# annappo/GPS-SDR-Receiver

Measured on AMD Instinct MI355X. Metric: IQ Msamples/s ingested, 32-SV acq + 12-ch track, higher is better.
Workload: dtype f32

## Files before the change

### gps-sdr-receiver_amd/csrc/gpsmi_fft.h

```cpp
#pragma once
#include <hip/hip_runtime.h>

namespace gpsmi {

__device__ __forceinline__ void lds_barrier() {
    asm volatile("s_waitcnt lgkmcnt(0)\n\ts_barrier" ::: "memory");
}


constexpr int kFftN = 2048;
constexpr int kFftThreads = 256;
constexpr int kFftPlane = kFftN + kFftN / 32;
constexpr int kFftPlane1 = kFftN + 8 * (kFftN / 64);
constexpr int kFftLdsFloats = 2 * kFftPlane + 2 * kFftPlane1;

__device__ __forceinline__ int fft_pad(int i) { return i + (i >> 5); }
__device__ __forceinline__ int fft_pad1(int i) { return i + 8 * (i >> 6); }

typedef float fft_c __attribute__((ext_vector_type(2)));

__device__ __forceinline__ fft_c cadd_mi(fft_c a, fft_c b) {
    fft_c d;
    asm("v_pk_add_f32 %0, %1, %2 op_sel:[0,1] op_sel_hi:[1,0] neg_hi:[0,1]" : "=v"(d) : "v"(a), "v"(b));
    return d;
}
__device__ __forceinline__ fft_c cadd_pi(fft_c a, fft_c b) {
    fft_c d;
    asm("v_pk_add_f32 %0, %1, %2 op_sel:[0,1] op_sel_hi:[1,0] neg_lo:[0,1]" : "=v"(d) : "v"(a), "v"(b));
    return d;
}
__device__ __forceinline__ fft_c cneg_add_mi(fft_c a) {
    fft_c d;
    asm("v_pk_add_f32 %0, %1, %1 op_sel:[0,1] op_sel_hi:[1,0] neg_lo:[1,0] neg_hi:[1,1]" : "=v"(d) : "v"(a));
    return d;
}
__device__ __forceinline__ fft_c cmulp(fft_c a, fft_c w) {
    fft_c d;
    asm("v_pk_mul_f32 %0, %2, %1 op_sel_hi:[1,0]\n\t"
        "v_pk_fma_f32 %0, %2, %1, %0 op_sel:[1,1,0] op_sel_hi:[0,1,1] neg_lo:[1,0,0]"
        : "=&v"(d) : "v"(a), "v"(w));
    return d;
}

__device__ __forceinline__ fft_c cmulp_conj(fft_c a, fft_c w) {
    fft_c d;
    asm("v_pk_mul_f32 %0, %2, %1 op_sel_hi:[1,0]\n\t"
        "v_pk_fma_f32 %0, %2, %1, %0 op_sel:[1,1,0] op_sel_hi:[0,1,1] neg_hi:[1,0,0]"
        : "=&v"(d) : "v"(a), "v"(w));
    return d;
}

template <bool B2MI>
__device__ __forceinline__ void dft4p(fft_c& b0, fft_c& b1, fft_c& b2, fft_c& b3) {
    const fft_c c0 = B2MI ? cadd_mi(b0, b2) : b0 + b2;
    const fft_c c1 = B2MI ? cadd_pi(b0, b2) : b0 - b2;
    const fft_c c2 = b1 + b3, d = b1 - b3;
    b0 = c0 + c2;
    b2 = c0 - c2;
    b1 = cadd_mi(c1, d);
    b3 = cadd_pi(c1, d);
}

__device__ __forceinline__ void dft8p(fft_c* v) {
    const float h = 0.70710678118654752440f;
    fft_c a0 = v[0] + v[4], a4 = v[0] - v[4];
    fft_c a1 = v[1] + v[5], a5 = v[1] - v[5];
    fft_c a2 = v[2] + v[6], a6 = v[2] - v[6];
    fft_c a3 = v[3] + v[7], a7 = v[3] - v[7];
    a5 = cadd_mi(a5, a5) * h;
    a7 = cneg_add_mi(a7) * h;
    dft4p<false>(a0, a1, a2, a3);
    dft4p<true>(a4, a5, a6, a7);
    v[0] = a0; v[2] = a1; v[4] = a2; v[6] = a3;
    v[1] = a4; v[3] = a5; v[5] = a6; v[7] = a7;
}

constexpr int kFftTwFloats = 2 * (64 + 512);
struct FftTw {
    const fft_c* t64;
    const fft_c* t512;
    fft_c w4[2][3];
};

__device__ __forceinline__ FftTw fft_setup(float* lds_tw, const float2* __restrict__ tw, int t) {
    float2* t64 = reinterpret_cast<float2*>(lds_tw);
    float2* t512 = t64 + 64;
    t64[t & 63] = tw[32 * (t & 63)];
    t512[t] = tw[4 * t];
    t512[t + 256] = tw[4 * (t + 256)];
    FftTw f;
    f.t64 = reinterpret_cast<const fft_c*>(t64);
    f.t512 = reinterpret_cast<const fft_c*>(t512);
#pragma unroll
    for (int b = 0; b < 2; ++b)
#pragma unroll
        for (int r = 1; r <= 3; ++r) {
            const float2 w = tw[r * (t + 256 * b)];
            f.w4[b][r - 1] = fft_c{w.x, w.y};
        }
    return f;
}

__device__ __forceinline__ void fft2048(float2* vio, float* lds, const FftTw& tw, int t) {
    fft_c* buf0 = reinterpret_cast<fft_c*>(lds);
    fft_c* buf1 = buf0 + kFftPlane;
    fft_c v[8];
#pragma unroll
    for (int r = 0; r < 8; ++r) v[r] = fft_c{vio[r].x, vio[r].y};

    dft8p(v);
#pragma unroll
    for (int r = 0; r < 8; ++r) buf0[fft_pad(8 * t + r)] = v[r];
    lds_barrier();
#pragma unroll
    for (int r = 0; r < 8; ++r) v[r] = buf0[fft_pad(t + 256 * r)];
    {
        const int k = t & 7;
#pragma unroll
        for (int r = 1; r < 8; ++r) v[r] = cmulp(v[r], tw.t64[r * k]);
        dft8p(v);
        const int base = (t >> 3) * 64 + k;
#pragma unroll
        for (int r = 0; r < 8; ++r) buf1[fft_pad1(base + 8 * r)] = v[r];
    }
    lds_barrier();
#pragma unroll
    for (int r = 0; r < 8; ++r) v[r] = buf1[fft_pad1(t + 256 * r)];
    {
        const int k = t & 63;
#pragma unroll
        for (int r = 1; r < 8; ++r) v[r] = cmulp(v[r], tw.t512[r * k]);
        dft8p(v);
        const int base = (t >> 6) * 512 + k;
#pragma unroll
        for (int r = 0; r < 8; ++r) buf0[fft_pad(base + 64 * r)] = v[r];
    }
    lds_barrier();
#pragma unroll
    for (int r = 0; r < 8; ++r) v[r] = buf0[fft_pad(t + 256 * r)];
#pragma unroll
    for (int b = 0; b < 2; ++b) {
        fft_c z1 = cmulp(v[b + 2], tw.w4[b][0]);
        fft_c z2 = cmulp(v[b + 4], tw.w4[b][1]);
        fft_c z3 = cmulp(v[b + 6], tw.w4[b][2]);
        fft_c z0 = v[b];
        dft4p<false>(z0, z1, z2, z3);
        v[b] = z0; v[b + 2] = z1; v[b + 4] = z2; v[b + 6] = z3;
    }
#pragma unroll
    for (int r = 0; r < 8; ++r) vio[r] = make_float2(v[r].x, v[r].y);
}

}
```

### gps-sdr-receiver_amd/csrc/gpsmi_stats.h

```cpp
#pragma once
#include <hip/hip_runtime.h>

#include "gpsmi_fft.h"

namespace gpsmi {

template <int CTRL, int ROWS>
__device__ __forceinline__ float dpp_add0(float v) {
    const float o = __builtin_bit_cast(
        float, __builtin_amdgcn_update_dpp(0, __builtin_bit_cast(int, v), CTRL, ROWS, 0xF, false));
    return v + o;
}
__device__ __forceinline__ float wave_sum_dpp(float v) {
    v = dpp_add0<0xB1, 0xF>(v);
    v = dpp_add0<0x4E, 0xF>(v);
    v = dpp_add0<0x141, 0xF>(v);
    v = dpp_add0<0x140, 0xF>(v);
    v = dpp_add0<0x142, 0xA>(v);
    v = dpp_add0<0x143, 0xC>(v);
    return __builtin_bit_cast(float, __builtin_amdgcn_readlane(__builtin_bit_cast(int, v), 63));
}

template <int CTRL>
__device__ __forceinline__ double dpp_add_f64(double v) {
    const long long b = __builtin_bit_cast(long long, v);
    const int lo = __builtin_amdgcn_update_dpp(0, (int)(b & 0xffffffffll), CTRL, 0xF, 0xF, false);
    const int hi = __builtin_amdgcn_update_dpp(0, (int)(b >> 32), CTRL, 0xF, 0xF, false);
    return v + __builtin_bit_cast(double, ((long long)hi << 32) | (unsigned)lo);
}
__device__ __forceinline__ double row_sum_f64_dpp(double v) {
    v = dpp_add_f64<0xB1>(v);
    v = dpp_add_f64<0x4E>(v);
    v = dpp_add_f64<0x141>(v);
    v = dpp_add_f64<0x140>(v);
    return v;
}

template <int CTRL, int ROWS>
__device__ __forceinline__ float dpp_max_own(float v) {
    const int vi = __builtin_bit_cast(int, v);
    return fmaxf(v, __builtin_bit_cast(float, __builtin_amdgcn_update_dpp(vi, vi, CTRL, ROWS, 0xF, false)));
}
template <int CTRL, int ROWS>
__device__ __forceinline__ int dpp_min_own(int v) {
    return min(v, __builtin_amdgcn_update_dpp(v, v, CTRL, ROWS, 0xF, false));
}
__device__ __forceinline__ void wave_argmax_dpp(float& v, int& i) {
    float m = v;
    m = dpp_max_own<0xB1, 0xF>(m);
    m = dpp_max_own<0x4E, 0xF>(m);
    m = dpp_max_own<0x141, 0xF>(m);
    m = dpp_max_own<0x140, 0xF>(m);
    m = dpp_max_own<0x142, 0xA>(m);
    m = dpp_max_own<0x143, 0xC>(m);
    m = __builtin_bit_cast(float, __builtin_amdgcn_readlane(__builtin_bit_cast(int, m), 63));
    int k = v == m ? i : 0x7fffffff;
    k = dpp_min_own<0xB1, 0xF>(k);
    k = dpp_min_own<0x4E, 0xF>(k);
    k = dpp_min_own<0x141, 0xF>(k);
    k = dpp_min_own<0x140, 0xF>(k);
    k = dpp_min_own<0x142, 0xA>(k);
    k = dpp_min_own<0x143, 0xC>(k);
    v = m;
    i = __builtin_amdgcn_readlane(k, 63);
}

constexpr int kStatsRedFloats = 16;

__device__ __forceinline__ void corr_stats8(const float* mag, int t, float* magbuf, float* red,
                                            int& amax, float& peak, float& mean, float& sd,
                                            float& lo, float& hi) {
    constexpr int N = 2048;
    const int wave = t >> 6, lane = t & 63;
    float sm = 0.f, bv = mag[0];
    int bi = t;
#pragma unroll
    for (int q = 0; q < 8; ++q) {
        sm += mag[q];
        if (mag[q] > bv) { bv = mag[q]; bi = t + 256 * q; }
        magbuf[t + 256 * q] = mag[q];
    }
    sm = wave_sum_dpp(sm);
    wave_argmax_dpp(bv, bi);
    if (lane == 0) { red[wave] = sm; red[4 + wave] = bv; ((int*)red)[8 + wave] = bi; }
    lds_barrier();
    sm = (red[0] + red[1]) + (red[2] + red[3]);
    bv = red[4]; bi = ((int*)red)[8];
#pragma unroll
    for (int w = 1; w < 4; ++w) {
        const float ov = red[4 + w];
        const int oi = ((int*)red)[8 + w];
        if (ov > bv || (ov == bv && oi < bi)) { bv = ov; bi = oi; }
    }
    mean = sm * (1.0f / N);
    float d2 = 0.f;
#pragma unroll
    for (int q = 0; q < 8; ++q) { const float d = mag[q] - mean; d2 += d * d; }
    d2 = wave_sum_dpp(d2);
    if (lane == 0) red[12 + wave] = d2;
    lds_barrier();
    d2 = (red[12] + red[13]) + (red[14] + red[15]);
    sd = sqrtf(d2 * (1.0f / N));
    amax = bi;
    peak = bv;
    lo = magbuf[(bi + N - 1) & (N - 1)];
    hi = magbuf[(bi + 1) & (N - 1)];
}

}
```

### gps-sdr-receiver_amd/csrc/gpsmi_trk.hip

```cpp
#include <atomic>
#include <chrono>
#include <cmath>
#include <condition_variable>
#include <cstdlib>
#include <cstring>
#include <deque>
#include <mutex>
#include <thread>
#include <vector>

#include <hip/hip_ext.h>

#include "gpsmi_common.h"
#include "gpsmi_fft.h"

#pragma clang fp contract(off)

namespace gpsmi {

constexpr float kTwoPiF = 6.28318530717958647692f;
constexpr float kPiF = 3.14159265358979323846f;

struct TrkParams {
    int cs;
// ... 663 lines not shown
    float2* d_rep = nullptr;
    float* d_code = nullptr;
    bool have_rep[GPSMI_MAX_PRN + 1] = {};
    float2* d_block = nullptr;
    gpsmi_trk_state* d_state = nullptr;
    std::vector<gpsmi_trk_state> h_state;
    bool state_dirty_host = false;
    size_t njobs_cap = 0;
    gpsmi_trk_state* d_tab_in = nullptr;
    gpsmi_trk_state* d_tab_out = nullptr;
    int* d_forced = nullptr;
    float last_total_ms = 0.f, last_corr_ms = 0.f, last_cp_ms = 0.f;
    int replay_nb = 0;
    bool replay_forced = false;
    int corr_cg = 4;
    int corr_small1 = 384, corr_small2 = 1536;
    int done_by_dispatch = 1;
    bool general = false;
    static constexpr int stream_j = 8;
    int mfma = 0;
    int codephase = 0;
    int corr_overlap = 0;
    int fold_chunk = 0;
    int epilogue_form = 1;
    float* d_code_eo = nullptr;
    int n_cu = 256;
    int iq_fmt = GPSMI_IQ_C64;
    int nchunks = 1;
    float2* d_fold = nullptr; float* d_mag = nullptr; DirStats* d_stats = nullptr;
    int* d_xsel = nullptr; int* d_rsel = nullptr; float2* d_partial_g = nullptr;
    bool big = false;
    float2* d_twN = nullptr; float2* d_RS = nullptr; float2* d_S = nullptr;
    bool pfa = false;
    float2* d_RSp = nullptr;
    bool span8 = false;
    TrkParams P;
    struct StreamJob { const void* iq; size_t n; gpsmi_trk_out* out; };
    struct StreamWorker {
        std::thread th;
        std::mutex m;
        std::condition_variable cv_job, cv_done;
        std::deque<StreamJob> q;
        bool stop = false;
        long long submitted = 0;
        long long cleared = 0;
        long long finished = 0;
        std::atomic<long long> a_submitted{0}, a_cleared{0}, a_finished{0};
        int err = 0;
        char errmsg[512] = "";
    };
    StreamWorker* worker = nullptr;
    int stream_thread = 1;
    int stream_depth = 2;
    long long stat_backlog = 0;
    long long stat_quiesce_ns = 0, stat_evwait_ns = 0, stat_waits = 0;
    long long stat_wait_ns = 0, stat_launch_ns = 0, stat_steps = 0;
};

constexpr int kSpanUnitsMax = 256;

static int trk_reserve(gpsmi_trk* h, size_t njobs) {
    if (njobs <= h->njobs_cap) return GPSMI_OK;
    void* olds[] = {h->d_tab_in, h->d_tab_out, h->d_forced, h->slot[0].d_mid, h->slot[1].d_mid,
                    h->slot[0].d_partial, h->slot[1].d_partial, h->slot[0].d_out, h->slot[1].d_out,
                    h->d_fold, h->d_mag, h->d_stats, h->d_xsel, h->d_rsel, h->d_partial_g,
                    h->slot[0].d_rec, h->slot[1].d_rec};
    for (void* p : olds)
        if (p) GPSMI_HIP(hipFree(p));
    h->d_tab_in = h->d_tab_out = nullptr; h->d_forced = nullptr;
    for (auto& sl : h->slot) { sl.d_mid = nullptr; sl.d_partial = nullptr; sl.d_out = nullptr; sl.d_rec = nullptr; }
    h->njobs_cap = 0;
    h->d_fold = nullptr; h->d_mag = nullptr; h->d_stats = nullptr; h->d_xsel = h->d_rsel = nullptr;
    h->d_partial_g = nullptr;
    if (h->mfma == 4)
        for (auto& sl : h->slot)
            GPSMI_HIP(hipMalloc((void**)&sl.d_rec, (size_t)kSpanUnitsMax * 32 * kSpRecFloats * sizeof(float)));
    if (h->general) {
        const size_t cs = h->cfg.code_samples;
        GPSMI_HIP(hipMalloc((void**)&h->d_fold, njobs * cs * sizeof(float2)));
        if (!h->pfa) GPSMI_HIP(hipMalloc((void**)&h->d_mag, njobs * cs * sizeof(float)));
        GPSMI_HIP(hipMalloc((void**)&h->d_stats, njobs * sizeof(DirStats)));
        GPSMI_HIP(hipMalloc((void**)&h->d_xsel, njobs * sizeof(int)));
        GPSMI_HIP(hipMalloc((void**)&h->d_rsel, njobs * sizeof(int)));
    }
    if (h->span8) {
        const size_t units = ((njobs + h->max_ch - 1) / h->max_ch) * ((h->max_ch + kSpCh - 1) / kSpCh);
        for (auto& sl : h->slot)
            GPSMI_HIP(hipMalloc((void**)&sl.d_rec, units * kS8Ranges * kS8RecFloats * sizeof(float)));
    }
    if (h->nchunks > 1 && !h->span8)
        GPSMI_HIP(hipMalloc((void**)&h->d_partial_g,
                            njobs * h->nchunks * (h->cfg.n_cyc + 1) * sizeof(float2)));
    GPSMI_HIP(hipMalloc((void**)&h->d_tab_in, njobs * sizeof(gpsmi_trk_state)));
    GPSMI_HIP(hipMalloc((void**)&h->d_tab_out, njobs * sizeof(gpsmi_trk_state)));
    GPSMI_HIP(hipMalloc((void**)&h->d_forced, njobs * sizeof(int)));
    for (auto& sl : h->slot) {
        GPSMI_HIP(hipMalloc((void**)&sl.d_mid, njobs * sizeof(JobMid)));
        GPSMI_HIP(hipMalloc((void**)&sl.d_partial, njobs * (h->cfg.n_cyc + 1) * sizeof(float2)));
        GPSMI_HIP(hipMalloc((void**)&sl.d_out, njobs * sizeof(gpsmi_trk_out)));
    }
    h->njobs_cap = njobs;
    return GPSMI_OK;
}

static int trk_launch(gpsmi_trk* h, gpsmi_trk::Slot& sl, const void* d_iq_v,
                      const gpsmi_trk_state* st_in, gpsmi_trk_state* st_out, const int* forced,
                      int njobs, int nch, bool side_epilogue = false, hipEvent_t tail_stop = nullptr,
                      bool* tail_stop_used = nullptr) {
    TrkParams P = h->P;
    P.nch = nch;
    hipStream_t rs = sl.run_stream ? sl.run_stream : h->stream;
    h->main_tail = nullptr;
    const float2* d_iq = static_cast<const float2*>(d_iq_v);
    const bool u8 = h->iq_fmt == GPSMI_IQ_U8;
    sl.corr_stop = sl.ev[2];
    const bool timed = h->timing == 1;
    const bool corr_stamps = h->timing == 2;
    if (timed) GPSMI_HIP(hipEventRecord(sl.ev[0], rs));
    const int nblocks = njobs / nch;
    const int ngroups = (nch + kGroupCh - 1) / kGroupCh;
    const dim3 sgrid(((nblocks + 7) / 8) * 8 * ngroups);
    const int ng_span = (nch + kSpCh - 1) / kSpCh;
    const bool span_single = h->mfma == 4 && nblocks * ng_span <= h->span_single_max;
    if (h->general) {
        const int cs = P.cs;
        const int chunk = (h->pfa && h->fold_chunk > 0 && h->fold_chunk < nblocks) ? h->fold_chunk : nblocks;
        for (int b0 = 0; b0 < nblocks; b0 += chunk) {
            const int nbc = nblocks - b0 < chunk ? nblocks - b0 : chunk;
            hipLaunchKernelGGL(trk_fold_general_kernel, dim3((cs + 255) / 256, nbc), dim3(256), 0,
                               rs, d_iq, h->d_t32, st_in, P, h->d_fold, h->d_xsel, h->d_rsel,
                               sl.d_mid, b0);
            if (h->pfa)
                pfa_corr_launch(rs, h->d_fold, h->d_xsel, h->d_rsel, nbc * nch, h->d_RSp, h->d_stats, b0 * nch);
        }
        if (h->pfa) {
        } else if (h->big)
            big_corr_launch(rs, h->d_fold, h->d_xsel, h->d_rsel, njobs, cs, h->d_RS, h->d_S,
                            h->d_tw, h->d_twN, h->d_mag);
        else
            hipLaunchKernelGGL(circ_corr_direct_kernel,
                               dim3((cs + kDirLagsPerWg - 1) / kDirLagsPerWg, njobs), dim3(256), 0,
                               rs, h->d_fold, h->d_code, h->d_xsel, h->d_rsel, cs,
                               h->d_mag);
        if (!h->pfa)
            hipLaunchKernelGGL(corr_stats_kernel, dim3(njobs), dim3(256), 0, rs, h->d_mag, cs,
                               h->d_stats);
        hipLaunchKernelGGL(trk_decide_kernel, dim3((njobs + 255) / 256), dim3(256), 0, rs,
                           h->d_stats, forced, P, njobs, sl.d_out, sl.d_mid);
    } else {
        const int jobs_all = nblocks * nch;
        const int cg = jobs_all <= h->corr_small1 ? 1 : (jobs_all <= h->corr_small2 ? 2 : h->corr_cg);
        const int ng = (nch + cg - 1) / cg;
        const dim3 cgrid(corr_grid(nblocks, ng));
#define GPSMI_LAUNCH_CORR(CGV)                                                                          \
    do {                                                                                              \
        if (u8)                                                                                       \
            hipLaunchKernelGGL((trk_corr_kernel<CGV, 1>), cgrid, dim3(256), 0, rs, d_iq_v,     \
                               st_in, forced, h->d_rep, h->d_tw, P, ng, nblocks, sl.d_out, sl.d_mid); \
        else                                                                                          \
            hipLaunchKernelGGL((trk_corr_kernel<CGV, 0>), cgrid, dim3(256), 0, rs, d_iq_v,     \
                               st_in, forced, h->d_rep, h->d_tw, P, ng, nblocks, sl.d_out, sl.d_mid); \
    } while (0)
        if (cg == 6) GPSMI_LAUNCH_CORR(6);
        else if (cg == 4) GPSMI_LAUNCH_CORR(4);
        else if (cg == 2) GPSMI_LAUNCH_CORR(2);
        else GPSMI_LAUNCH_CORR(1);
#undef GPSMI_LAUNCH_CORR
    }
    const bool ext_timed = (timed || corr_stamps) && h->mfma == 4 && !span_single;
    bool corr_done_recorded = false;
    const int span_units = nblocks * ng_span, span_slots = sp_wg_per_cu(P.n_cyc) * h->n_cu;
    const int span_per = (span_units + span_slots - 1) / span_slots;
    const dim3 span_grid((span_units + span_per - 1) / (span_per > 0 ? span_per : 1));
    if (timed && !ext_timed) GPSMI_HIP(hipEventRecord(sl.ev[1], rs));
    if (h->mfma) {
        const int ng12 = (nch + kSpCh - 1) / kSpCh;
        const JobMid* cmid = sl.d_mid;
        const float* ceo = h->d_code_eo;
#define GPSMI_LAUNCH_SPAN(NSP, WV, FMTV, NCV, GRID, BLOCK)                                                     \
    do {                                                                                                      \
        if (ext_timed && (NSP) == 8)                                                                          \
            hipExtLaunchKernelGGL((trk_span_kernel<NSP, WV, FMTV, 0, NCV>), GRID, BLOCK, 0, rs, sl.ev[1],     \
                                  sl.corr_stop, 0, d_iq_v, cmid, ceo, P, ng12, nblocks, sl.d_rec,             \
                                  sl.d_partial);                                                              \
        else if (by_dispatch && (NSP) == 8)                                                                   \
            hipExtLaunchKernelGGL((trk_span_kernel<NSP, WV, FMTV, 0, NCV>), GRID, BLOCK, 0, rs, nullptr,      \
                                  sl.corr_done, 0, d_iq_v, cmid, ceo, P, ng12, nblocks, sl.d_rec,             \
                                  sl.d_partial);                                                              \
        else                                                                                                  \
            hipLaunchKernelGGL((trk_span_kernel<NSP, WV, FMTV, 0, NCV>), GRID, BLOCK, 0, rs, d_iq_v, cmid,    \
                               ceo, P, ng12, nblocks, sl.d_rec, sl.d_partial);                                \
    } while (0)
#define GPSMI_LAUNCH_SPAN_NC(NCV)                                                                       \
    do {                                                                                               \
        if (span_single && u8) GPSMI_LAUNCH_SPAN(1, 1, 1, NCV, dim3(nblocks * ng12 * 32), dim3(64));   \
        else if (span_single) GPSMI_LAUNCH_SPAN(1, 1, 0, NCV, dim3(nblocks * ng12 * 32), dim3(64));    \
        else if (u8) GPSMI_LAUNCH_SPAN(8, 4, 1, NCV, span_grid, dim3(256));                            \
        else GPSMI_LAUNCH_SPAN(8, 4, 0, NCV, span_grid, dim3(256));                                    \
    } while (0)
        const bool by_dispatch = !span_single && side_epilogue && h->done_by_dispatch;
        sl.corr_stop = (ext_timed && by_dispatch) ? sl.corr_done : sl.ev[2];
        if (P.n_cyc == 32) GPSMI_LAUNCH_SPAN_NC(32);
        else if (P.n_cyc == 16) GPSMI_LAUNCH_SPAN_NC(16);
        else GPSMI_LAUNCH_SPAN_NC(8);
#undef GPSMI_LAUNCH_SPAN_NC
#undef GPSMI_LAUNCH_SPAN
        corr_done_recorded = by_dispatch;
    } else if (h->span8) {
        const int ng12 = (nch + kSpCh - 1) / kSpCh;
        const int nwaves = nblocks * ng12 * kS8Ranges;
        hipLaunchKernelGGL(trk_span8_kernel, dim3((nwaves + 3) / 4), dim3(256), 0, rs, d_iq,
                           sl.d_mid, h->d_code_eo, P, ng12, nblocks, sl.d_rec);
    } else {
        const dim3 grid(sgrid.x, h->nchunks), block(kStreamThreads);
        float2* pdst = h->nchunks > 1 ? h->d_partial_g : sl.d_partial;
#define GPSMI_LAUNCH_STREAM(NC, POW2, J)                                                        \
    hipLaunchKernelGGL((trk_stream_kernel<NC, POW2, J>), grid, block, 0, rs, d_iq, st_in, \
                       sl.d_mid, h->d_code, P, ngroups, nblocks, pdst)
#define GPSMI_LAUNCH_STREAM_NC(POW2, J)                 \
    do {                                                \
        if (P.n_cyc == 32) GPSMI_LAUNCH_STREAM(32, POW2, J);      \
        else if (P.n_cyc == 16) GPSMI_LAUNCH_STREAM(16, POW2, J); \
        else GPSMI_LAUNCH_STREAM(8, POW2, J);           \
    } while (0)
        if (h->general) GPSMI_LAUNCH_STREAM_NC(false, 8);
        else GPSMI_LAUNCH_STREAM_NC(true, 8);
#undef GPSMI_LAUNCH_STREAM_NC
#undef GPSMI_LAUNCH_STREAM
        if (h->nchunks > 1) {
            const int per_job = P.n_cyc + 1;
            hipLaunchKernelGGL(trk_partial_reduce_kernel, dim3((njobs * per_job + 255) / 256),
                               dim3(256), 0, rs, h->d_partial_g, h->nchunks, per_job, njobs,
                               sl.d_mid, sl.d_partial);
        }
    }
    if (timed && !ext_timed) GPSMI_HIP(hipEventRecord(sl.ev[2], rs));
    hipStream_t es = rs;
    if (side_epilogue) {
        es = h->epi_stream;
        if (!corr_done_recorded) GPSMI_HIP(hipEventRecord(sl.corr_done, rs));
        h->main_tail = sl.corr_done;
        GPSMI_HIP(hipStreamWaitEvent(es, sl.corr_done, 0));
    }
    const gpsmi_trk_state* c_in = st_in;
    const JobMid* c_mid = sl.d_mid;
    const float* c_rec = sl.d_rec;
    const float2* c_partial = sl.d_partial;
    bool stop_used = false;
#define GPSMI_LAUNCH_EPI_SPAN(NCV)                                                                         \
    do {                                                                                                  \
        if (tail_stop) {                                                                                  \
            hipExtLaunchKernelGGL(trk_epilogue_span_kernel<NCV>, dim3(njobs), dim3(256), 0, es, nullptr,  \
                                  tail_stop, 0, c_in, st_out, c_mid, c_rec, ng_span, P, njobs, sl.d_out); \
            stop_used = true;                                                                             \
        } else {                                                                                          \
            hipLaunchKernelGGL(trk_epilogue_span_kernel<NCV>, dim3(njobs), dim3(256), 0, es, c_in,        \
                               st_out, c_mid, c_rec, ng_span, P, njobs, sl.d_out);                        \
        }                                                                                                 \
    } while (0)
    if (h->span8)
        hipLaunchKernelGGL(trk_epilogue_span8_kernel, dim3((njobs + 3) / 4), dim3(256), 0, es, st_in,
                           st_out, sl.d_mid, sl.d_rec, ng_span, P, njobs, sl.d_out);
    else if (span_single && P.n_cyc == 32)
        GPSMI_LAUNCH_EPI_SPAN(32);
    else if (span_single && P.n_cyc == 16)
        GPSMI_LAUNCH_EPI_SPAN(16);
    else if (span_single)
        GPSMI_LAUNCH_EPI_SPAN(8);
    else if (h->epilogue_form == 0) {
        if (tail_stop) {
            hipExtLaunchKernelGGL(trk_epilogue_kernel, dim3((njobs + 3) / 4), dim3(256), 0, es, nullptr,
                                  tail_stop, 0, c_in, st_out, c_mid, c_partial, P, njobs, sl.d_out);
            stop_used = true;
        } else
            hipLaunchKernelGGL(trk_epilogue_kernel, dim3((njobs + 3) / 4), dim3(256), 0, es, st_in,
                               st_out, sl.d_mid, sl.d_partial, P, njobs, sl.d_out);
    } else {
#define GPSMI_LAUNCH_EPI8(NCV)                                                                           \
    do {                                                                                                \
        if (tail_stop) {                                                                                \
            hipExtLaunchKernelGGL(trk_epilogue8_kernel<NCV>, dim3((njobs + 7) / 8), dim3(64), 0, es,    \
                                  nullptr, tail_stop, 0, c_in, st_out, c_mid, c_partial, P, njobs,      \
                                  sl.d_out);                                                            \
            stop_used = true;                                                                           \
        } else {                                                                                        \
            hipLaunchKernelGGL(trk_epilogue8_kernel<NCV>, dim3((njobs + 7) / 8), dim3(64), 0, es, c_in, \
                               st_out, c_mid, c_partial, P, njobs, sl.d_out);                           \
        }                                                                                               \
    } while (0)
        if (P.n_cyc == 32) GPSMI_LAUNCH_EPI8(32);
        else if (P.n_cyc == 16) GPSMI_LAUNCH_EPI8(16);
        else GPSMI_LAUNCH_EPI8(8);
#undef GPSMI_LAUNCH_EPI8
    }
#undef GPSMI_LAUNCH_EPI_SPAN
    if (tail_stop_used) *tail_stop_used = stop_used;
    GPSMI_HIP(hipGetLastError());
    if (timed) GPSMI_HIP(hipEventRecord(sl.ev[3], es));
    if (side_epilogue) {
        GPSMI_HIP(hipEventRecord(sl.epi_done, es));
        sl.epi_pending = true;
    }
    return GPSMI_OK;
}

namespace gpsmi {
HandleSync acq_sync(gpsmi_acq* h);
HandleSync trk_sync(gpsmi_trk* h);
}

static int trk_take_timing(gpsmi_trk* h, gpsmi_trk::Slot& sl) {
    if (!sl.timing_pending) return GPSMI_OK;
    if (sl.timing_pending == 1) {
        GPSMI_HIP(hipEventElapsedTime(&h->last_total_ms, sl.ev[0], sl.ev[3]));
        GPSMI_HIP(hipEventElapsedTime(&h->last_cp_ms, sl.ev[0], sl.ev[1]));
    }
    GPSMI_HIP(hipEventElapsedTime(&h->last_corr_ms, sl.ev[1], sl.corr_stop ? sl.corr_stop : sl.ev[2]));
    sl.timing_pending = 0;
    return GPSMI_OK;
}
// ... 965 lines not shown
```

### gps-sdr-receiver_amd/csrc/gpsmi_trk_corr.h

```cpp
#pragma once
#include <type_traits>
#include "gpsmi_fft.h"
#include "gpsmi_stats.h"
#include "gpsmi_wgmap.h"

namespace gpsmi {

template <int CG> constexpr int kFoldDepthOf = CG == 1 ? 8 : 3;
constexpr int kFoldChunk = 8;

struct CorrFin { int bi; float bv, mean, sd, elo, ehi; };

__device__ __forceinline__ void corr_finish(const StreamChan& s, const CorrFin& f, const TrkParams& P,
                                            const int* __restrict__ delay_forced,
                                            gpsmi_trk_out* __restrict__ out, JobMid* __restrict__ mid) {
    const int bi = f.bi;
    const float bv = f.bv, mean = f.mean, sd = f.sd, elo = f.elo, ehi = f.ehi;
    const float norm = (bv - mean) / sd;
    gpsmi_trk_out& o = out[s.job];
    o.prn = s.prn;
    o.mx = bi;
    o.epl[0] = elo; o.epl[1] = bv; o.epl[2] = ehi;
    o.corr_mean = mean; o.corr_std = sd;
    o.norm_max_corr = norm;
    int delay = -1;
    double cp = -1.0;
    if (norm > P.corr_min) {
        delay = bi;
        cp = fit_code_phase((double)elo, (double)bv, (double)ehi, bi);
    }
    o.delay = delay;
    o.reserved0 = 0;
    o.code_phase = cp;
    int used = delay >= 0 ? delay : s.d;
    if (delay_forced && delay_forced[s.job] >= 0) used = delay_forced[s.job];
    o.delay_used = used;
    JobMid md;
    md.delay_used = used; md.active = 1; md.prn = s.prn; md.om = s.om; md.ph = s.ph;
    md.pad[0] = md.pad[1] = md.pad[2] = 0;
    mid[s.job] = md;
}

template <int CG, int FMT = 0>
__global__ __launch_bounds__(256, (CG > 4 || CG == 1) ? 2 : 3) void trk_corr_kernel(
    const void* __restrict__ iq, const gpsmi_trk_state* __restrict__ st_in,
    const int* __restrict__ delay_forced, const float2* __restrict__ rep,
    const float2* __restrict__ tw, TrkParams P, int ngroups, int nblocks,
    gpsmi_trk_out* __restrict__ out, JobMid* __restrict__ mid) {
    __shared__ __attribute__((aligned(16))) float lds[kFftLdsFloats];
    __shared__ __attribute__((aligned(16))) float lds_tw[kFftTwFloats];
    __shared__ float red[kStatsRedFloats];
    float* magbuf = lds + 2 * kFftPlane;
    float2 (*urow)[32] = reinterpret_cast<float2 (*)[32]>(lds + 2 * kFftPlane);
    float2 (*vtab)[32] = urow + CG;
    float2* step = reinterpret_cast<float2*>(urow + 2 * CG);
    static_assert(kFftN <= 2 * kFftPlane1 && (CG * 64 + CG) * 2 <= 2 * kFftPlane1, "aliases must fit buffer 1");
    __shared__ StreamChan schan[CG];
    __shared__ CorrFin fin[CG];

    const CorrWg unit = corr_wg_map((int)blockIdx.x, nblocks, ngroups);
    const int g = unit.group, b = unit.block;
    if (b >= nblocks) return;
    const int t = threadIdx.x;
    const int cs = kFftN;
    constexpr int kFoldDepth = kFoldDepthOf<CG>;
    const float2* blk = static_cast<const float2*>(iq) + (size_t)b * ((size_t)cs * P.n_cyc);
    const uint16_t* rblk = static_cast<const uint16_t*>(iq) + (size_t)b * ((size_t)cs * P.n_cyc);
    const double inv_2pi = 0.15915494309189533576888376337251;
    const int first = (P.n_cyc - P.corr_avg) / 2;
    const int pc_c = min(t / 33, CG - 1);
    const gpsmi_trk_state& st = st_in[b * P.nch + min(g * CG + pc_c, P.nch - 1)];
    int st_prn = st.prn, st_delay = st.delay;
    float st_om0 = st.omega0, st_freq = st.freq, st_phase = st.phase;
    using Raw = typename std::conditional<FMT == 0, v2f, unsigned>::type;
    auto fetch = [&](int i, int r) -> Raw {
        if constexpr (FMT == 0) {
            const float2 v = blk[(size_t)i * cs + t + 256 * r];
            return v2f{v.x, v.y};
        } else {
            return (unsigned)rblk[(size_t)i * cs + t + 256 * r];
        }
    };
    auto decode = [&](Raw v) -> v2f {
        if constexpr (FMT == 0) {
            return v;
        } else {
            const float scl = 1.0f / 127.5f;
            return v2f{sub_rn(mul_rn((float)(v & 0xFF), scl), 1.0f), sub_rn(mul_rn((float)(v >> 8), scl), 1.0f)};
        }
    };
    Raw x[kFoldDepth][8];
    const bool nofold = diag_flag(P, 32);
    const bool piped = P.corr_avg == kFoldChunk && !nofold;
    if (piped) {
#pragma unroll
        for (int k = 0; k < kFoldDepth; ++k)
#pragma unroll
            for (int r = 0; r < 8; ++r) x[k][r] = fetch(first + k, r);
    }
    const FftTw ftw = fft_setup(lds_tw, tw, t);
    asm volatile("" : "+v"(st_prn), "+v"(st_delay), "+v"(st_om0), "+v"(st_freq), "+v"(st_phase));

    if (t < CG * 33) {
        const int c = t / 33, i = t % 33;
        const int cidx = g * CG + c;
        const int job = b * P.nch + cidx;
        StreamChan s;
        s.job = job; s.active = 0; s.om = 0.f; s.ph = 0.f; s.d = 0; s.prn = 0;
        if (cidx < P.nch && st_prn > 0) {
            s.active = 1;
            s.om = st_om0 != 0.f ? st_om0 : omega_of(st_freq);
            s.ph = st_phase;
            s.d = st_delay;
            s.prn = st_prn;
        }
        const double f_eff = (double)s.om * inv_2pi;
        if (i < 32) {
            const double rev = f_eff * (double)i * 1.0e-3;
            urow[c][i] = phasor_rev((float)(rev - rint(rev)));
            const double per = f_eff / (1000.0 * (double)cs);
            const double rv = i < 16 ? per * (double)(i + 1) + (double)s.ph * inv_2pi
                                     : per * (double)(16 * (i - 16));
            vtab[c][i] = phasor_rev((float)(rv - rint(rv)));
        } else {
            const double rev = f_eff * 256.0 / (1000.0 * (double)cs);
            step[c] = phasor_rev((float)(rev - rint(rev)));
            schan[c] = s;
            if (cidx < P.nch && !s.active) {
                JobMid z;
                z.delay_used = 0; z.active = 0; z.prn = 0; z.om = 0.f; z.ph = 0.f;
                z.pad[0] = z.pad[1] = z.pad[2] = 0;
                mid[job] = z;
            }
        }
    }
    lds_barrier();

    v2f acc[CG][8];
#pragma unroll
    for (int c = 0; c < CG; ++c)
#pragma unroll
        for (int r = 0; r < 8; ++r) acc[c][r] = v2f{0.f, 0.f};
    auto fold_in = [&](const v2f (&u)[CG], int r, v2f xr, v2f xprev) {
        if constexpr (CG == 1) {
            if (r & 1) cmac2(acc[0][r - 1], acc[0][r], u[0], xprev, u[0], xr);
        } else {
#pragma unroll
            for (int c = 0; c + 1 < CG; c += 2)
                cmac2(acc[c][r], acc[c + 1][r], u[c], xr, u[c + 1], xr);
        }
    };
    auto fold_row = [&](int i, Raw (&xk)[8], auto reload, int inext) {
        v2f u[CG];
#pragma unroll
        for (int c = 0; c < CG; ++c) u[c] = v2f{urow[c][i].x, urow[c][i].y};
        v2f xprev = v2f{0.f, 0.f};
#pragma unroll
        for (int r = 0; r < 8; ++r) {
            const v2f xr = decode(xk[r]);
            fold_in(u, r, xr, xprev);
            xprev = xr;
            if constexpr (decltype(reload)::value) {
                if (CG > 1 || (r & 1)) {
                    xk[r] = fetch(inext, r);
                    if (CG == 1) xk[r - 1] = fetch(inext, r - 1);
                }
            }
        }
    };
    if (piped) {
#pragma unroll
        for (int j = 0; j < kFoldChunk; ++j) {
            if (j + kFoldDepth < kFoldChunk)
                fold_row(first + j, x[j % kFoldDepth], std::true_type{}, first + j + kFoldDepth);
            else
                fold_row(first + j, x[j % kFoldDepth], std::false_type{}, 0);
            __builtin_amdgcn_sched_barrier(0);
        }
    } else if (!nofold) {
        for (int i = first; i < first + P.corr_avg; ++i) {
#pragma unroll
            for (int r = 0; r < 8; ++r) x[0][r] = fetch(i, r);
            fold_row(i, x[0], std::false_type{}, 0);
        }
    }

    const float sc = (1.0f / (float)P.corr_avg) * (1.0f / kFftN);
#pragma unroll
    for (int c = 0; c < CG; ++c) {
        const float2 e1 = vtab[c][t & 15], e2 = vtab[c][16 + (t >> 4)], s2 = step[c];
        fft_c vm = cmulp(fft_c{e1.x, e1.y}, fft_c{e2.x, e2.y});
        const fft_c st256 = fft_c{s2.x, s2.y};
#pragma unroll
        for (int r = 0; r < 8; ++r) {
            acc[c][r] = cmulp(acc[c][r] * sc, vm);
            vm = cmulp(vm, st256);
        }
    }
    auto prepare = [&](int c, const StreamChan& s, float2 (&v)[8], float2 (&rs)[8]) {
#pragma unroll
        for (int r = 0; r < 8; ++r) v[r] = make_float2(acc[c][r].x, acc[c][r].y);
        const float2* R = rep + (size_t)s.prn * kFftN;
#pragma unroll
        for (int q = 0; q < 8; ++q) rs[q] = R[t + 256 * q];
    };
    auto times_conj = [&](float2 (&v)[8], const float2 (&rs)[8]) {
#pragma unroll
        for (int q = 0; q < 8; ++q) {
            const fft_c o = cmulp_conj(fft_c{v[q].x, v[q].y}, fft_c{rs[q].x, rs[q].y});
            v[q] = make_float2(o.x, o.y);
        }
    };
    auto magnitudes = [&](const float2 (&v)[8], float (&mag)[8]) {
#pragma unroll
        for (int q = 0; q < 8; ++q)
            mag[q] = __builtin_amdgcn_sqrtf(v[q].x * v[q].x + v[q].y * v[q].y);
    };
    auto single = [&](int c) {
        const StreamChan s = schan[c];
        float2 v[8], rs[8];
        prepare(c, s, v, rs);
        fft2048(v, lds, ftw, t);
        times_conj(v, rs);
        lds_barrier();
        fft2048(v, lds, ftw, t);
        float mag[8];
        magnitudes(v, mag);
        int bi; float bv, mean, sd, elo, ehi;
        corr_stats8(mag, t, magbuf, red, bi, bv, mean, sd, elo, ehi);
        if (t == 0) fin[c] = CorrFin{bi, bv, mean, sd, elo, ehi};
    };
    if (diag_flag(P, 64)) {
        float sm = 0.f;
#pragma unroll
        for (int c = 0; c < CG; ++c)
#pragma unroll
            for (int r = 0; r < 8; ++r) sm += acc[c][r].x + acc[c][r].y;
        if (t < CG && schan[t].active)
            corr_finish(schan[t], CorrFin{0, sm, 0.f, 1.f, 0.f, 0.f}, P, delay_forced, out, mid);
        return;
    }
#pragma unroll
    for (int c = 0; c < CG; ++c)
        if (schan[c].active) single(c);
    __syncthreads();
    if (t < CG && schan[t].active) corr_finish(schan[t], fin[t], P, delay_forced, out, mid);
}

}
```

Baseline: 288,900.

## Batch correlation stats across channels and compact FFT twiddle tables

After: 286,900. No clear change (-0.7%).

```diff
diff --git a/gps-sdr-receiver_amd/csrc/gpsmi_fft.h b/gps-sdr-receiver_amd/csrc/gpsmi_fft.h
--- a/gps-sdr-receiver_amd/csrc/gpsmi_fft.h
+++ b/gps-sdr-receiver_amd/csrc/gpsmi_fft.h
@@ -75,7 +75,8 @@
     v[1] = a4; v[3] = a5; v[5] = a6; v[7] = a7;
 }
 
-constexpr int kFftTwFloats = 2 * (64 + 512);
+constexpr int kFftTw64 = 7 * 8, kFftTw512 = 7 * 64;
+constexpr int kFftTwFloats = 2 * (kFftTw64 + kFftTw512);
 struct FftTw {
     const fft_c* t64;
     const fft_c* t512;
@@ -84,13 +85,15 @@
 
 __device__ __forceinline__ FftTw fft_setup(float* lds_tw, const float2* __restrict__ tw, int t) {
     float2* t64 = reinterpret_cast<float2*>(lds_tw);
-    float2* t512 = t64 + 64;
-    t64[t & 63] = tw[32 * (t & 63)];
-    t512[t] = tw[4 * t];
-    t512[t + 256] = tw[4 * (t + 256)];
+    float2* t512 = t64 + kFftTw64;
+    const int i64 = min(t & 63, kFftTw64 - 1);
+    t64[i64] = tw[32 * ((i64 >> 3) + 1) * (i64 & 7)];
+    t512[t] = tw[4 * ((t >> 6) + 1) * (t & 63)];
+    const int i512 = min(t + 256, kFftTw512 - 1);
+    t512[i512] = tw[4 * ((i512 >> 6) + 1) * (i512 & 63)];
     FftTw f;
-    f.t64 = reinterpret_cast<const fft_c*>(t64);
-    f.t512 = reinterpret_cast<const fft_c*>(t512);
+    f.t64 = reinterpret_cast<const fft_c*>(t64) + (t & 7);
+    f.t512 = reinterpret_cast<const fft_c*>(t512) + (t & 63);
 #pragma unroll
     for (int b = 0; b < 2; ++b)
 #pragma unroll
@@ -101,12 +104,9 @@
     return f;
 }
 
-__device__ __forceinline__ void fft2048(float2* vio, float* lds, const FftTw& tw, int t) {
+__device__ __forceinline__ void fft2048(fft_c (&v)[8], float* lds, const FftTw& tw, int t) {
     fft_c* buf0 = reinterpret_cast<fft_c*>(lds);
     fft_c* buf1 = buf0 + kFftPlane;
-    fft_c v[8];
-#pragma unroll
-    for (int r = 0; r < 8; ++r) v[r] = fft_c{vio[r].x, vio[r].y};
 
     dft8p(v);
 #pragma unroll
@@ -117,7 +117,7 @@
     {
         const int k = t & 7;
 #pragma unroll
-        for (int r = 1; r < 8; ++r) v[r] = cmulp(v[r], tw.t64[r * k]);
+        for (int r = 1; r < 8; ++r) v[r] = cmulp(v[r], tw.t64[8 * (r - 1)]);
         dft8p(v);
         const int base = (t >> 3) * 64 + k;
 #pragma unroll
@@ -129,7 +129,7 @@
     {
         const int k = t & 63;
 #pragma unroll
-        for (int r = 1; r < 8; ++r) v[r] = cmulp(v[r], tw.t512[r * k]);
+        for (int r = 1; r < 8; ++r) v[r] = cmulp(v[r], tw.t512[64 * (r - 1)]);
         dft8p(v);
         const int base = (t >> 6) * 512 + k;
 #pragma unroll
@@ -147,6 +147,13 @@
         dft4p<false>(z0, z1, z2, z3);
         v[b] = z0; v[b + 2] = z1; v[b + 4] = z2; v[b + 6] = z3;
     }
+}
+
+__device__ __forceinline__ void fft2048(float2* vio, float* lds, const FftTw& tw, int t) {
+    fft_c v[8];
+#pragma unroll
+    for (int r = 0; r < 8; ++r) v[r] = fft_c{vio[r].x, vio[r].y};
+    fft2048(v, lds, tw, t);
 #pragma unroll
     for (int r = 0; r < 8; ++r) vio[r] = make_float2(v[r].x, v[r].y);
 }
diff --git a/gps-sdr-receiver_amd/csrc/gpsmi_stats.h b/gps-sdr-receiver_amd/csrc/gpsmi_stats.h
--- a/gps-sdr-receiver_amd/csrc/gpsmi_stats.h
+++ b/gps-sdr-receiver_amd/csrc/gpsmi_stats.h
@@ -5,6 +5,11 @@
 
 namespace gpsmi {
 
+template <int CTRL>
+__device__ __forceinline__ float dpp_add_all(float v) {
+    const int vi = __builtin_bit_cast(int, v);
+    return v + __builtin_bit_cast(float, __builtin_amdgcn_update_dpp(vi, vi, CTRL, 0xF, 0xF, true));
+}
 template <int CTRL, int ROWS>
 __device__ __forceinline__ float dpp_add0(float v) {
     const float o = __builtin_bit_cast(
@@ -12,10 +17,10 @@
     return v + o;
 }
 __device__ __forceinline__ float wave_sum_dpp(float v) {
-    v = dpp_add0<0xB1, 0xF>(v);
-    v = dpp_add0<0x4E, 0xF>(v);
-    v = dpp_add0<0x141, 0xF>(v);
-    v = dpp_add0<0x140, 0xF>(v);
+    v = dpp_add_all<0xB1>(v);
+    v = dpp_add_all<0x4E>(v);
+    v = dpp_add_all<0x141>(v);
+    v = dpp_add_all<0x140>(v);
     v = dpp_add0<0x142, 0xA>(v);
     v = dpp_add0<0x143, 0xC>(v);
     return __builtin_bit_cast(float, __builtin_amdgcn_readlane(__builtin_bit_cast(int, v), 63));
@@ -36,6 +41,15 @@
     return v;
 }
 
+template <int CTRL>
+__device__ __forceinline__ float dpp_max_all(float v) {
+    const int vi = __builtin_bit_cast(int, v);
+    return fmaxf(v, __builtin_bit_cast(float, __builtin_amdgcn_update_dpp(vi, vi, CTRL, 0xF, 0xF, true)));
+}
+template <int CTRL>
+__device__ __forceinline__ int dpp_min_all(int v) {
+    return min(v, __builtin_amdgcn_update_dpp(v, v, CTRL, 0xF, 0xF, true));
+}
 template <int CTRL, int ROWS>
 __device__ __forceinline__ float dpp_max_own(float v) {
     const int vi = __builtin_bit_cast(int, v);
@@ -47,18 +61,18 @@
 }
 __device__ __forceinline__ void wave_argmax_dpp(float& v, int& i) {
     float m = v;
-    m = dpp_max_own<0xB1, 0xF>(m);
-    m = dpp_max_own<0x4E, 0xF>(m);
-    m = dpp_max_own<0x141, 0xF>(m);
-    m = dpp_max_own<0x140, 0xF>(m);
+    m = dpp_max_all<0xB1>(m);
+    m = dpp_max_all<0x4E>(m);
+    m = dpp_max_all<0x141>(m);
+    m = dpp_max_all<0x140>(m);
     m = dpp_max_own<0x142, 0xA>(m);
     m = dpp_max_own<0x143, 0xC>(m);
     m = __builtin_bit_cast(float, __builtin_amdgcn_readlane(__builtin_bit_cast(int, m), 63));
     int k = v == m ? i : 0x7fffffff;
-    k = dpp_min_own<0xB1, 0xF>(k);
-    k = dpp_min_own<0x4E, 0xF>(k);
-    k = dpp_min_own<0x141, 0xF>(k);
-    k = dpp_min_own<0x140, 0xF>(k);
+    k = dpp_min_all<0xB1>(k);
+    k = dpp_min_all<0x4E>(k);
+    k = dpp_min_all<0x141>(k);
+    k = dpp_min_all<0x140>(k);
     k = dpp_min_own<0x142, 0xA>(k);
     k = dpp_min_own<0x143, 0xC>(k);
     v = m;
@@ -107,4 +121,93 @@
     hi = magbuf[(bi + 1) & (N - 1)];
 }
 
-}
+constexpr int kStatsBatchFloats = 20;
+template <int NC>
+__device__ __forceinline__ void corr_stats8_batch(const float (&mag)[NC][8], int t, float* red) {
+    constexpr int N = 2048;
+    const int wave = t >> 6, lane = t & 63;
+    float sm[NC], bv[NC];
+    int bi[NC];
+#pragma unroll
+    for (int c = 0; c < NC; ++c) {
+        sm[c] = 0.f; bv[c] = mag[c][0]; bi[c] = t;
+#pragma unroll
+        for (int q = 0; q < 8; ++q) {
+            sm[c] += mag[c][q];
+            if (mag[c][q] > bv[c]) { bv[c] = mag[c][q]; bi[c] = t + 256 * q; }
+        }
+    }
+#pragma unroll
+    for (int c = 0; c < NC; ++c) {
+        sm[c] = wave_sum_dpp(sm[c]);
+        wave_argmax_dpp(bv[c], bi[c]);
+    }
+    if (lane == 0) {
+#pragma unroll
+        for (int c = 0; c < NC; ++c) {
+            float* r = red + kStatsBatchFloats * c;
+            r[wave] = sm[c]; r[4 + wave] = bv[c]; ((int*)r)[8 + wave] = bi[c];
+        }
+    }
+    lds_barrier();
+    float d2[NC];
+#pragma unroll
+    for (int c = 0; c < NC; ++c) {
+        const float* r = red + kStatsBatchFloats * c;
+        const float mean = ((r[0] + r[1]) + (r[2] + r[3])) * (1.0f / N);
+        d2[c] = 0.f;
+#pragma unroll
+        for (int q = 0; q < 8; ++q) { const float d = mag[c][q] - mean; d2[c] += d * d; }
+        float pv = r[4];
+        int pi = ((const int*)r)[8];
+#pragma unroll
+        for (int w = 1; w < 4; ++w) {
+            const float ov = r[4 + w];
+            const int oi = ((const int*)r)[8 + w];
+            if (ov > pv || (ov == pv && oi < pi)) { pv = ov; pi = oi; }
+        }
+        bi[c] = pi;
+    }
+#pragma unroll
+    for (int c = 0; c < NC; ++c) d2[c] = wave_sum_dpp(d2[c]);
+#pragma unroll
+    for (int c = 0; c < NC; ++c) {
+        float* r = red + kStatsBatchFloats * c;
+        if (lane == 0) r[12 + wave] = d2[c];
+#pragma unroll
+        for (int side = 0; side < 2; ++side) {
+            const int lag = (bi[c] + (side ? 1 : N - 1)) & (N - 1);
+            if ((lag & 255) == t) {
+                const int ql = lag >> 8;
+                float m = mag[c][0];
+#pragma unroll
+                for (int q = 1; q < 8; ++q) m = ql == q ? mag[c][q] : m;
+                r[16 + side] = m;
+            }
+        }
+    }
+}
+
+__device__ __forceinline__ void corr_stats_fetch(const float* red, int c, int& amax, float& peak,
+                                                 float& mean, float& sd, float& lo, float& hi) {
+    constexpr int N = 2048;
+    const float* r = red + kStatsBatchFloats * c;
+    const float sm = (r[0] + r[1]) + (r[2] + r[3]);
+    float bv = r[4];
+    int bi = ((const int*)r)[8];
+#pragma unroll
+    for (int w = 1; w < 4; ++w) {
+        const float ov = r[4 + w];
+        const int oi = ((const int*)r)[8 + w];
+        if (ov > bv || (ov == bv && oi < bi)) { bv = ov; bi = oi; }
+    }
+    mean = sm * (1.0f / N);
+    const float d2 = (r[12] + r[13]) + (r[14] + r[15]);
+    sd = sqrtf(d2 * (1.0f / N));
+    amax = bi;
+    peak = bv;
+    lo = r[16];
+    hi = r[17];
+}
+
+}
diff --git a/gps-sdr-receiver_amd/csrc/gpsmi_trk.hip b/gps-sdr-receiver_amd/csrc/gpsmi_trk.hip
--- a/gps-sdr-receiver_amd/csrc/gpsmi_trk.hip
+++ b/gps-sdr-receiver_amd/csrc/gpsmi_trk.hip
@@ -839,20 +839,28 @@
         const int cg = jobs_all <= h->corr_small1 ? 1 : (jobs_all <= h->corr_small2 ? 2 : h->corr_cg);
         const int ng = (nch + cg - 1) / cg;
         const dim3 cgrid(corr_grid(nblocks, ng));
+#define GPSMI_LAUNCH_CORR_P(CGV, KERNEL)                                                                \
+    do {                                                                                              \
+        if (u8)                                                                                       \
+            hipLaunchKernelGGL((KERNEL<CGV, 1>), cgrid, dim3(256), 0, rs, d_iq_v,                     \
+                               st_in, forced, h->d_rep, h->d_tw, P, ng, nblocks, sl.d_out, sl.d_mid); \
+        else                                                                                          \
+            hipLaunchKernelGGL((KERNEL<CGV, 0>), cgrid, dim3(256), 0, rs, d_iq_v,                     \
+                               st_in, forced, h->d_rep, h->d_tw, P, ng, nblocks, sl.d_out, sl.d_mid); \
+    } while (0)
 #define GPSMI_LAUNCH_CORR(CGV)                                                                          \
     do {                                                                                              \
-        if (u8)                                                                                       \
-            hipLaunchKernelGGL((trk_corr_kernel<CGV, 1>), cgrid, dim3(256), 0, rs, d_iq_v,     \
-                               st_in, forced, h->d_rep, h->d_tw, P, ng, nblocks, sl.d_out, sl.d_mid); \
+        if (P.corr_avg == kFoldChunk)          \
+            GPSMI_LAUNCH_CORR_P(CGV, trk_corr_kernel);                                                            \
         else                                                                                          \
-            hipLaunchKernelGGL((trk_corr_kernel<CGV, 0>), cgrid, dim3(256), 0, rs, d_iq_v,     \
-                               st_in, forced, h->d_rep, h->d_tw, P, ng, nblocks, sl.d_out, sl.d_mid); \
+            GPSMI_LAUNCH_CORR_P(CGV, trk_corr_rows_kernel);                                                           \
     } while (0)
         if (cg == 6) GPSMI_LAUNCH_CORR(6);
         else if (cg == 4) GPSMI_LAUNCH_CORR(4);
         else if (cg == 2) GPSMI_LAUNCH_CORR(2);
         else GPSMI_LAUNCH_CORR(1);
 #undef GPSMI_LAUNCH_CORR
+#undef GPSMI_LAUNCH_CORR_P
     }
     const bool ext_timed = (timed || corr_stamps) && h->mfma == 4 && !span_single;
     bool corr_done_recorded = false;
diff --git a/gps-sdr-receiver_amd/csrc/gpsmi_trk_corr.h b/gps-sdr-receiver_amd/csrc/gpsmi_trk_corr.h
--- a/gps-sdr-receiver_amd/csrc/gpsmi_trk_corr.h
+++ b/gps-sdr-receiver_amd/csrc/gpsmi_trk_corr.h
@@ -41,22 +41,20 @@
     mid[s.job] = md;
 }
 
-template <int CG, int FMT = 0>
-__global__ __launch_bounds__(256, (CG > 4 || CG == 1) ? 2 : 3) void trk_corr_kernel(
+template <int CG, int FMT, bool PIPED>
+__device__ __forceinline__ void trk_corr_body(
     const void* __restrict__ iq, const gpsmi_trk_state* __restrict__ st_in,
     const int* __restrict__ delay_forced, const float2* __restrict__ rep,
     const float2* __restrict__ tw, TrkParams P, int ngroups, int nblocks,
     gpsmi_trk_out* __restrict__ out, JobMid* __restrict__ mid) {
     __shared__ __attribute__((aligned(16))) float lds[kFftLdsFloats];
     __shared__ __attribute__((aligned(16))) float lds_tw[kFftTwFloats];
-    __shared__ float red[kStatsRedFloats];
-    float* magbuf = lds + 2 * kFftPlane;
-    float2 (*urow)[32] = reinterpret_cast<float2 (*)[32]>(lds + 2 * kFftPlane);
-    float2 (*vtab)[32] = urow + CG;
-    float2* step = reinterpret_cast<float2*>(urow + 2 * CG);
+    __shared__ __attribute__((aligned(16))) float red[kStatsBatchFloats * CG];
+    v2f (*urow)[32] = reinterpret_cast<v2f (*)[32]>(lds + 2 * kFftPlane);
+    v2f (*vtab)[32] = urow + CG;
+    v2f* step = reinterpret_cast<v2f*>(urow + 2 * CG);
     static_assert(kFftN <= 2 * kFftPlane1 && (CG * 64 + CG) * 2 <= 2 * kFftPlane1, "aliases must fit buffer 1");
     __shared__ StreamChan schan[CG];
-    __shared__ CorrFin fin[CG];
 
     const CorrWg unit = corr_wg_map((int)blockIdx.x, nblocks, ngroups);
     const int g = unit.group, b = unit.block;
@@ -64,7 +62,7 @@
     const int t = threadIdx.x;
     const int cs = kFftN;
     constexpr int kFoldDepth = kFoldDepthOf<CG>;
-    const float2* blk = static_cast<const float2*>(iq) + (size_t)b * ((size_t)cs * P.n_cyc);
+    const v2f* blk = static_cast<const v2f*>(iq) + (size_t)b * ((size_t)cs * P.n_cyc);
     const uint16_t* rblk = static_cast<const uint16_t*>(iq) + (size_t)b * ((size_t)cs * P.n_cyc);
     const double inv_2pi = 0.15915494309189533576888376337251;
     const int first = (P.n_cyc - P.corr_avg) / 2;
@@ -75,8 +73,7 @@
     using Raw = typename std::conditional<FMT == 0, v2f, unsigned>::type;
     auto fetch = [&](int i, int r) -> Raw {
         if constexpr (FMT == 0) {
-            const float2 v = blk[(size_t)i * cs + t + 256 * r];
-            return v2f{v.x, v.y};
+            return blk[(size_t)i * cs + t + 256 * r];
         } else {
             return (unsigned)rblk[(size_t)i * cs + t + 256 * r];
         }
@@ -91,7 +88,7 @@
     };
     Raw x[kFoldDepth][8];
     const bool nofold = diag_flag(P, 32);
-    const bool piped = P.corr_avg == kFoldChunk && !nofold;
+    const bool piped = PIPED && !nofold;
     if (piped) {
 #pragma unroll
         for (int k = 0; k < kFoldDepth; ++k)
@@ -117,14 +114,17 @@
         const double f_eff = (double)s.om * inv_2pi;
         if (i < 32) {
             const double rev = f_eff * (double)i * 1.0e-3;
-            urow[c][i] = phasor_rev((float)(rev - rint(rev)));
+            const float2 u = phasor_rev((float)(rev - rint(rev)));
+            urow[c][i] = v2f{u.x, u.y};
             const double per = f_eff / (1000.0 * (double)cs);
             const double rv = i < 16 ? per * (double)(i + 1) + (double)s.ph * inv_2pi
                                      : per * (double)(16 * (i - 16));
-            vtab[c][i] = phasor_rev((float)(rv - rint(rv)));
+            const float2 e = phasor_rev((float)(rv - rint(rv)));
+            vtab[c][i] = v2f{e.x, e.y};
         } else {
             const double rev = f_eff * 256.0 / (1000.0 * (double)cs);
-            step[c] = phasor_rev((float)(rev - rint(rev)));
+            const float2 e = phasor_rev((float)(rev - rint(rev)));
+            step[c] = v2f{e.x, e.y};
             schan[c] = s;
             if (cidx < P.nch && !s.active) {
                 JobMid z;
@@ -153,7 +153,7 @@
     auto fold_row = [&](int i, Raw (&xk)[8], auto reload, int inext) {
         v2f u[CG];
 #pragma unroll
-        for (int c = 0; c < CG; ++c) u[c] = v2f{urow[c][i].x, urow[c][i].y};
+        for (int c = 0; c < CG; ++c) u[c] = urow[c][i];
         v2f xprev = v2f{0.f, 0.f};
 #pragma unroll
         for (int r = 0; r < 8; ++r) {
@@ -168,7 +168,8 @@
             }
         }
     };
-    if (piped) {
+    if constexpr (PIPED) {
+        if (piped) {
 #pragma unroll
         for (int j = 0; j < kFoldChunk; ++j) {
             if (j + kFoldDepth < kFoldChunk)
@@ -177,6 +178,7 @@
                 fold_row(first + j, x[j % kFoldDepth], std::false_type{}, 0);
             __builtin_amdgcn_sched_barrier(0);
         }
+        }
     } else if (!nofold) {
         for (int i = first; i < first + P.corr_avg; ++i) {
 #pragma unroll
@@ -188,47 +190,29 @@
     const float sc = (1.0f / (float)P.corr_avg) * (1.0f / kFftN);
 #pragma unroll
     for (int c = 0; c < CG; ++c) {
-        const float2 e1 = vtab[c][t & 15], e2 = vtab[c][16 + (t >> 4)], s2 = step[c];
-        fft_c vm = cmulp(fft_c{e1.x, e1.y}, fft_c{e2.x, e2.y});
-        const fft_c st256 = fft_c{s2.x, s2.y};
+        fft_c vm = cmulp(vtab[c][t & 15], vtab[c][16 + (t >> 4)]);
+        const fft_c st256 = step[c];
 #pragma unroll
         for (int r = 0; r < 8; ++r) {
             acc[c][r] = cmulp(acc[c][r] * sc, vm);
             vm = cmulp(vm, st256);
         }
     }
-    auto prepare = [&](int c, const StreamChan& s, float2 (&v)[8], float2 (&rs)[8]) {
-#pragma unroll
-        for (int r = 0; r < 8; ++r) v[r] = make_float2(acc[c][r].x, acc[c][r].y);
-        const float2* R = rep + (size_t)s.prn * kFftN;
+    float mag[CG][8];
+    auto single = [&](int c) {
+        const fft_c* R = reinterpret_cast<const fft_c*>(rep) + (size_t)schan[c].prn * kFftN;
+        fft_c rs[8];
 #pragma unroll
         for (int q = 0; q < 8; ++q) rs[q] = R[t + 256 * q];
-    };
-    auto times_conj = [&](float2 (&v)[8], const float2 (&rs)[8]) {
-#pragma unroll
-        for (int q = 0; q < 8; ++q) {
-            const fft_c o = cmulp_conj(fft_c{v[q].x, v[q].y}, fft_c{rs[q].x, rs[q].y});
-            v[q] = make_float2(o.x, o.y);
-        }
-    };
-    auto magnitudes = [&](const float2 (&v)[8], float (&mag)[8]) {
+        fft2048(acc[c], lds, ftw, t);
+#pragma unroll
+        for (int q = 0; q < 8; ++q) acc[c][q] = cmulp_conj(acc[c][q], rs[q]);
+        lds_barrier();
+        fft2048(acc[c], lds, ftw, t);
 #pragma unroll
         for (int q = 0; q < 8; ++q)
-            mag[q] = __builtin_amdgcn_sqrtf(v[q].x * v[q].x + v[q].y * v[q].y);
-    };
-    auto single = [&](int c) {
-        const StreamChan s = schan[c];
-        float2 v[8], rs[8];
-        prepare(c, s, v, rs);
-        fft2048(v, lds, ftw, t);
-        times_conj(v, rs);
+            mag[c][q] = __builtin_amdgcn_sqrtf(acc[c][q].x * acc[c][q].x + acc[c][q].y * acc[c][q].y);
         lds_barrier();
-        fft2048(v, lds, ftw, t);
-        float mag[8];
-        magnitudes(v, mag);
-        int bi; float bv, mean, sd, elo, ehi;
-        corr_stats8(mag, t, magbuf, red, bi, bv, mean, sd, elo, ehi);
-        if (t == 0) fin[c] = CorrFin{bi, bv, mean, sd, elo, ehi};
     };
     if (diag_flag(P, 64)) {
         float sm = 0.f;
@@ -240,11 +224,39 @@
             corr_finish(schan[t], CorrFin{0, sm, 0.f, 1.f, 0.f, 0.f}, P, delay_forced, out, mid);
         return;
     }
-#pragma unroll
-    for (int c = 0; c < CG; ++c)
-        if (schan[c].active) single(c);
-    __syncthreads();
-    if (t < CG && schan[t].active) corr_finish(schan[t], fin[t], P, delay_forced, out, mid);
-}
-
-}
+    bool any = false;
+#pragma unroll
+    for (int c = 0; c < CG; ++c) {
+#pragma unroll
+        for (int q = 0; q < 8; ++q) mag[c][q] = 0.f;
+        if (schan[c].active) { single(c); any = true; }
+    }
+    if (!any) return;
+    corr_stats8_batch<CG>(mag, t, red);
+    lds_barrier();
+    if (t < CG && schan[t].active) {
+        CorrFin f;
+        corr_stats_fetch(red, t, f.bi, f.bv, f.mean, f.sd, f.elo, f.ehi);
+        corr_finish(schan[t], f, P, delay_forced, out, mid);
+    }
+}
+
+template <int CG, int FMT = 0>
+__global__ __launch_bounds__(256, (CG > 4 || CG == 1) ? 2 : 3) void trk_corr_kernel(
+    const void* __restrict__ iq, const gpsmi_trk_state* __restrict__ st_in,
+    const int* __restrict__ delay_forced, const float2* __restrict__ rep,
+    const float2* __restrict__ tw, TrkParams P, int ngroups, int nblocks,
+    gpsmi_trk_out* __restrict__ out, JobMid* __restrict__ mid) {
+    trk_corr_body<CG, FMT, true>(iq, st_in, delay_forced, rep, tw, P, ngroups, nblocks, out, mid);
+}
+
+template <int CG, int FMT = 0>
+__global__ __launch_bounds__(256, (CG > 4 || CG == 1) ? 2 : 3) void trk_corr_rows_kernel(
+    const void* __restrict__ iq, const gpsmi_trk_state* __restrict__ st_in,
+    const int* __restrict__ delay_forced, const float2* __restrict__ rep,
+    const float2* __restrict__ tw, TrkParams P, int ngroups, int nblocks,
+    gpsmi_trk_out* __restrict__ out, JobMid* __restrict__ mid) {
+    trk_corr_body<CG, FMT, false>(iq, st_in, delay_forced, rep, tw, P, ngroups, nblocks, out, mid);
+}
+
+}
```
